# nameofuser1/vad

Hardware: NVIDIA B200
Metric: audio_seconds_per_second (higher is better)
Workload: dtype f32

## Files before the change

### vad_b200/csrc/ffn_tc.cuh

```cuda
#pragma once

#include <cuda_fp16.h>
#include <cuda_runtime.h>

#include <algorithm>
#include <cmath>
#include <cstdint>
#include <cstring>
#include <vector>

#include "vad_core.cuh"

namespace vadb {

constexpr int kTcK1 = 48, kTcN1 = 64;
__host__ __device__ constexpr int tc_feat_col(int feat) {
  const int g = feat / 13, k = feat % 13, q = k / 2, e = k % 2;
  return q < 4 ? 6 * q + 2 * g + e : 24 + 6 * (q - 4) + 2 * g + e;
}
constexpr int kTcK2 = 64, kTcN2 = 32;
constexpr int kTcK3 = 32, kTcN3 = 16;
constexpr int kTcK4 = 16, kTcN4 = 16;
constexpr int kTcBlk1 = kTcK1 * kTcN1 * 4, kTcBlk2 = kTcK2 * kTcN2 * 4, kTcBlk3 = kTcK3 * kTcN3 * 4,
              kTcBlk4 = kTcK4 * kTcN4 * 4;
// ... 194 lines not shown
      "selp.u32 %0, 1, 0, p;\n\t}"
      : "=r"(ok)
      : "r"(tc_smem_u32(bar)), "r"(parity)
      : "memory");
  return ok != 0;
}
__device__ __forceinline__ void tc_mbar_wait(uint64_t* bar, uint32_t parity) {
  while (!tc_mbar_try_wait(bar, parity)) {
  }
}

__device__ __forceinline__ uint64_t tc_smem_desc(uint32_t smem_addr, uint32_t lbo_bytes, uint32_t sbo_bytes) {
  uint64_t d = 0;
  d |= static_cast<uint64_t>((smem_addr >> 4) & 0x3FFF);
  d |= static_cast<uint64_t>((lbo_bytes >> 4) & 0x3FFF) << 16;
  d |= static_cast<uint64_t>((sbo_bytes >> 4) & 0x3FFF) << 32;
  d |= 1ull << 46;
  return d;
}
__host__ __device__ constexpr uint32_t tc_idesc(int n) {
  return (1u << 4)  | (2u << 7)  | (2u << 10)  |
         (static_cast<uint32_t>(n >> 3) << 17) | (static_cast<uint32_t>(128 >> 4) << 24);
}

template <int K, int N>
__device__ __forceinline__ void tc_issue_layer(uint32_t tm_base, uint32_t d_col, uint32_t w_smem, uint64_t* done_bar) {
  constexpr uint32_t lbo = (2 * N / 8) * 128, sbo = 128;
  constexpr uint32_t idesc_2n = tc_idesc(2 * N), idesc_n = tc_idesc(N);
  const uint32_t a_hi = tm_base + kTmA, a_lo = tm_base + kTmA + K, d = tm_base + d_col;
#pragma unroll
  for (int j = 0; j < K / 8; ++j) {
    const uint64_t b = tc_smem_desc(w_smem + 2 * j * lbo, lbo, sbo);
    umma_tf32_ts(d, a_hi + 8 * j, b, idesc_2n, j > 0 ? 1u : 0u);
    umma_tf32_ts(d, a_lo + 8 * j, b, idesc_n, 1u);
  }
  umma_commit(done_bar);
}

__device__ __forceinline__ void tc_split(float x, uint32_t& hi, uint32_t& lo) {
  hi = __float_as_uint(x) & 0xFFFFE000u;
  lo = __float_as_uint(x - __uint_as_float(hi));
}

template <int NOUT, int HALVES>
__device__ __forceinline__ void tc_hidden_epilogue(uint32_t tl, uint32_t d_col, const float* bias, int hidx) {
  constexpr int W = NOUT / HALVES;
  constexpr int CH = W >= 16 ? 16 : 8;
  const int base = hidx * W;
#pragma unroll
  for (int c0 = 0; c0 < W; c0 += CH) {
    uint32_t v[CH], u[CH], hi[CH], lo[CH];
    if constexpr (CH == 16) {
      tmem_ld16(tl + d_col + base + c0, v);
      tmem_ld16(tl + d_col + NOUT + base + c0, u);
    } else {
      tmem_ld8(tl + d_col + base + c0, v);
      tmem_ld8(tl + d_col + NOUT + base + c0, u);
    }
    tmem_wait_ld();
#pragma unroll
    for (int i = 0; i < CH; ++i) {
      const float a = fmaxf((__uint_as_float(v[i]) + __uint_as_float(u[i])) + bias[base + c0 + i], 0.0f);
      tc_split(a, hi[i], lo[i]);
    }
    if constexpr (CH == 16) {
      tmem_st16(tl + kTmA + base + c0, hi);
      tmem_st16(tl + kTmA + NOUT + base + c0, lo);
    } else {
      tmem_st8(tl + kTmA + base + c0, hi);
      tmem_st8(tl + kTmA + NOUT + base + c0, lo);
    }
  }
  tmem_wait_st();
}

template <int HALVES>
__device__ __forceinline__ void tc_bar() {
  if constexpr (HALVES == 2) asm volatile("bar.sync 1, 256;" ::: "memory");
  else asm volatile("bar.sync 1, 128;" ::: "memory");
}

__device__ __forceinline__ void tc_store_a1_half(uint32_t tl, int hidx, const float (&xl)[24]) {
  uint32_t hi[16], lo[16], hi8[8], lo8[8];
#pragma unroll
  for (int i = 0; i < 16; ++i) tc_split(xl[i], hi[i], lo[i]);
#pragma unroll
  for (int i = 0; i < 8; ++i) tc_split(xl[16 + i], hi8[i], lo8[i]);
  const uint32_t b = tl + kTmA + 24 * hidx;
  tmem_st16(b, hi);
  tmem_st8(b + 16, hi8);
  tmem_st16(b + kTcK1, lo);
  tmem_st8(b + kTcK1 + 16, lo8);
}

template <int HALVES>
__device__ __forceinline__ uint32_t ffn_tc_tile(const FfnBias& fb, float (&logit)[kNCls], uint32_t tm_base, int wq, int hidx,
                                                bool is_issuer, uint32_t w_smem, uint64_t* mma_bar, uint32_t par,
                                                long long* ts = nullptr, int dbg = 0) {
  const uint32_t tl = tm_base + (static_cast<uint32_t>(32 * wq) << 16);
#define VADB_TS(i) do { if (ts) ts[i] = clock64(); } while (0)
  tmem_wait_st();
  tc_fence_before();
  tc_bar<HALVES>();
  VADB_TS(3);
  if (is_issuer && !(dbg & 32)) {
    tc_fence_after();
    tc_issue_layer<kTcK1, kTcN1>(tm_base, kTmD1, w_smem + kTcOff1, mma_bar);
  }
  VADB_TS(4);
  if (!(dbg & 32)) { tc_mbar_wait(mma_bar, par); par ^= 1u; }
  tc_fence_after();
  VADB_TS(5);
  if (!(dbg & 128)) tc_hidden_epilogue<kTcN1, HALVES>(tl, kTmD1, fb.b1, hidx);
  VADB_TS(6);
  tc_fence_before();
  tc_bar<HALVES>();
  if (is_issuer && !(dbg & 32)) {
    tc_fence_after();
    tc_issue_layer<kTcK2, kTcN2>(tm_base, kTmD2, w_smem + kTcOff2, mma_bar);
  }
  VADB_TS(7);
  if (!(dbg & 32)) { tc_mbar_wait(mma_bar, par); par ^= 1u; }
  tc_fence_after();
  VADB_TS(8);
  if (!(dbg & 128)) tc_hidden_epilogue<kTcN2, HALVES>(tl, kTmD2, fb.b2, hidx);
  VADB_TS(9);
  tc_fence_before();
  tc_bar<HALVES>();
  if (is_issuer && !(dbg & 32)) {
    tc_fence_after();
    tc_issue_layer<kTcK3, kTcN3>(tm_base, kTmD3, w_smem + kTcOff3, mma_bar);
  }
  VADB_TS(10);
  if (!(dbg & 32)) { tc_mbar_wait(mma_bar, par); par ^= 1u; }
  tc_fence_after();
  VADB_TS(11);
  if (!(dbg & 128)) tc_hidden_epilogue<kTcN3, HALVES>(tl, kTmD3, fb.b3, hidx);
  VADB_TS(12);
  tc_fence_before();
  tc_bar<HALVES>();
  if (is_issuer && !(dbg & 32)) {
    tc_fence_after();
    tc_issue_layer<kTcK4, kTcN4>(tm_base, kTmD4, w_smem + kTcOff4, mma_bar);
  }
  VADB_TS(13);
  if (!(dbg & 32)) { tc_mbar_wait(mma_bar, par); par ^= 1u; }
  tc_fence_after();
  VADB_TS(14);
  if (hidx == 0) {
    uint32_t v[8], u[8];
    tmem_ld8(tl + kTmD4, v);
    tmem_ld8(tl + kTmD4 + kTcN4, u);
    tmem_wait_ld();
#pragma unroll
    for (int o = 0; o < kNCls; ++o) logit[o] = (__uint_as_float(v[o]) + __uint_as_float(u[o])) + fb.b4[o];
  }
  tc_fence_before();
  VADB_TS(15);
#undef VADB_TS
  return par;
}

__device__ __forceinline__ void umma_f16_ts(uint32_t d_tmem, uint32_t a_tmem, uint64_t b_desc, uint32_t idesc,
                                            uint32_t accumulate) {
  asm volatile(
      "{\n\t.reg .pred p;\n\t"
      "setp.ne.b32 p, %4, 0;\n\t"
      "tcgen05.mma.cta_group::1.kind::f16 [%0], [%1], %2, %3, p;\n\t}" ::"r"(d_tmem),
      "r"(a_tmem), "l"(b_desc), "r"(idesc), "r"(accumulate)
      : "memory");
}
__host__ __device__ constexpr uint32_t tc16_idesc(int n) {
  return (1u << 4)  | (static_cast<uint32_t>(n >> 3) << 17) |
         (static_cast<uint32_t>(128 >> 4) << 24);
}
template <int K, int N>
__device__ __forceinline__ void tc16_issue_layer(uint32_t tm_base, uint32_t d_col, uint32_t w_smem, uint64_t* done_bar) {
  constexpr uint32_t lbo = (2 * N / 8) * 128, sbo = 128;
  constexpr uint32_t idesc_2n = tc16_idesc(2 * N), idesc_n = tc16_idesc(N);
  const uint32_t a_hi = tm_base + kTmA, a_lo = tm_base + kTmA + K / 2, d = tm_base + d_col;
#pragma unroll
  for (int j = 0; j < K / 16; ++j) {
    const uint64_t b = tc_smem_desc(w_smem + 2 * j * lbo, lbo, sbo);
    umma_f16_ts(d, a_hi + 8 * j, b, idesc_2n, j > 0 ? 1u : 0u);
    umma_f16_ts(d, a_lo + 8 * j, b, idesc_n, 1u);
  }
  umma_commit(done_bar);
}
__device__ __forceinline__ void tc16_split2(f2 x, uint32_t& hi, uint32_t& lo) {
  const __half2 h = __floats2half2_rn(x.x, x.y);
  const float2 hf = __half22float2(h);
  const f2 r = vsub(x, mk2(hf.x, hf.y));
  const __half2 l = __floats2half2_rn(r.x, r.y);
  hi = *reinterpret_cast<const uint32_t*>(&h);
  lo = *reinterpret_cast<const uint32_t*>(&l);
}
template <int NOUT, int HALVES>
__device__ __forceinline__ void tc16_hidden_epilogue(uint32_t tl, uint32_t d_col, const float* cbias, float postp,
                                                     int hidx) {
  constexpr int W = NOUT / HALVES;
  constexpr int CH = W >= 16 ? 16 : 8;
  const int base = hidx * W;
#pragma unroll
  for (int c0 = 0; c0 < W; c0 += CH) {
    uint32_t v[CH], u[CH], hi[CH / 2], lo[CH / 2];
    if constexpr (CH == 16) {
      tmem_ld16(tl + d_col + base + c0, v);
      tmem_ld16(tl + d_col + NOUT + base + c0, u);
    } else {
      tmem_ld8(tl + d_col + base + c0, v);
      tmem_ld8(tl + d_col + NOUT + base + c0, u);
    }
    tmem_wait_ld();
#pragma unroll
    for (int i = 0; i < CH; i += 2) {
      const f2 d = vadd(mk2(__uint_as_float(v[i]), __uint_as_float(v[i + 1])),
                        mk2(__uint_as_float(u[i]), __uint_as_float(u[i + 1])));
      f2 a = vfma(d, mk2(postp, postp), mk2(cbias[base + c0 + i], cbias[base + c0 + i + 1]));
      a.x = fmaxf(a.x, 0.0f);
      a.y = fmaxf(a.y, 0.0f);
      tc16_split2(a, hi[i / 2], lo[i / 2]);
    }
    if constexpr (CH == 16) {
      tmem_st8(tl + kTmA + (base + c0) / 2, hi);
      tmem_st8(tl + kTmA + NOUT / 2 + (base + c0) / 2, lo);
    } else {
      tmem_st4(tl + kTmA + (base + c0) / 2, hi);
      tmem_st4(tl + kTmA + NOUT / 2 + (base + c0) / 2, lo);
    }
  }
  tmem_wait_st();
}
__device__ __forceinline__ void tc16_store_a1_half(uint32_t tl, int hidx, const float (&xl)[24]) {
  uint32_t hi[8], lo[8], hi4[4], lo4[4];
#pragma unroll
  for (int i = 0; i < 8; ++i) tc16_split2(mk2(xl[2 * i], xl[2 * i + 1]), hi[i], lo[i]);
#pragma unroll
  for (int i = 0; i < 4; ++i) tc16_split2(mk2(xl[16 + 2 * i], xl[17 + 2 * i]), hi4[i], lo4[i]);
  const uint32_t b = tl + kTmA + 12 * hidx;
  tmem_st8(b, hi);
  tmem_st4(b + 8, hi4);
  tmem_st8(b + kTcK1 / 2, lo);
  tmem_st4(b + kTcK1 / 2 + 8, lo4);
}
template <int HALVES>
__device__ __forceinline__ uint32_t ffn_tc16_tile(const FfnBias& fb, float (&logit)[kNCls], uint32_t tm_base, int wq,
                                                  int hidx, bool is_issuer, uint32_t w_smem, uint64_t* mma_bar,
                                                  uint32_t par) {
  const uint32_t tl = tm_base + (static_cast<uint32_t>(32 * wq) << 16);
  tmem_wait_st();
  tc_fence_before();
  tc_bar<HALVES>();
  if (is_issuer) {
    tc_fence_after();
    tc16_issue_layer<kTcK1, kTcN1>(tm_base, kTmD1, w_smem + kTc16Off1, mma_bar);
  }
  tc_mbar_wait(mma_bar, par); par ^= 1u;
  tc_fence_after();
  tc16_hidden_epilogue<kTcN1, HALVES>(tl, kTmD1, fb.c1, fb.postp[0], hidx);
  tc_fence_before();
  tc_bar<HALVES>();
  if (is_issuer) {
    tc_fence_after();
    tc16_issue_layer<kTcK2, kTcN2>(tm_base, kTmD2, w_smem + kTc16Off2, mma_bar);
  }
  tc_mbar_wait(mma_bar, par); par ^= 1u;
  tc_fence_after();
  tc16_hidden_epilogue<kTcN2, HALVES>(tl, kTmD2, fb.c2, fb.postp[1], hidx);
  tc_fence_before();
  tc_bar<HALVES>();
  if (is_issuer) {
    tc_fence_after();
    tc16_issue_layer<kTcK3, kTcN3>(tm_base, kTmD3, w_smem + kTc16Off3, mma_bar);
  }
  tc_mbar_wait(mma_bar, par); par ^= 1u;
  tc_fence_after();
  tc16_hidden_epilogue<kTcN3, HALVES>(tl, kTmD3, fb.c3, fb.postp[2], hidx);
  tc_fence_before();
  tc_bar<HALVES>();
  if (is_issuer) {
    tc_fence_after();
    tc16_issue_layer<kTcK4, kTcN4>(tm_base, kTmD4, w_smem + kTc16Off4, mma_bar);
  }
  tc_mbar_wait(mma_bar, par); par ^= 1u;
  tc_fence_after();
  if (hidx == 0) {
    uint32_t v[8], u[8];
    tmem_ld8(tl + kTmD4, v);
    tmem_ld8(tl + kTmD4 + kTcN4, u);
    tmem_wait_ld();
#pragma unroll
    for (int o = 0; o < kNCls; ++o) logit[o] = fmaf(__uint_as_float(v[o]) + __uint_as_float(u[o]), fb.post[3], fb.b4[o]);
  }
  tc_fence_before();
  return par;
}

constexpr int kTm2Tile = 128;
constexpr int kTm2D1 = 64, kTm2D2 = 64, kTm2D3 = 64, kTm2D4 = 96;
static_assert(2 * kTm2Tile == kTmemCols && kTm2D1 + kTcN1 <= kTm2Tile && kTm2D2 + 2 * kTcN2 <= kTm2Tile &&
              kTm2D4 + 2 * kTcN4 <= kTm2Tile && kTcK2 <= kTm2D1, "two tiles share the CTA's TMEM allocation");

template <int K, int N, bool ONE_ACC>
__device__ __forceinline__ void tc16_issue_layer2(uint32_t tm_base, uint32_t d_col, uint32_t w_smem, bool two_tiles,
                                                  uint64_t* done_bar) {
  constexpr uint32_t lbo = (2 * N / 8) * 128, sbo = 128, lo_off = (N / 8) * 128;
  constexpr int kMmas = ONE_ACC ? 3 : 2;
#pragma unroll
  for (int j = 0; j < K / 16; ++j) {
    const uint32_t b = w_smem + 2 * j * lbo;
    const uint64_t b_hi = tc_smem_desc(b, lbo, sbo), b_lo = tc_smem_desc(b + lo_off, lbo, sbo);
#pragma unroll
    for (int m = 0; m < kMmas; ++m) {
      const uint32_t a_col = kTmA + (m == kMmas - 1 ? K / 2 : 0) + 8 * j;
      const uint64_t bd = (ONE_ACC && m == 1) ? b_lo : b_hi;
      const uint32_t idesc = (!ONE_ACC && m == 0) ? tc16_idesc(2 * N) : tc16_idesc(N);
      const uint32_t acc = (j > 0 || m > 0) ? 1u : 0u;
      umma_f16_ts(tm_base + d_col, tm_base + a_col, bd, idesc, acc);
      if (two_tiles) umma_f16_ts(tm_base + kTm2Tile + d_col, tm_base + kTm2Tile + a_col, bd, idesc, acc);
    }
  }
  umma_commit(done_bar);
}
template <int NOUT>
__device__ __forceinline__ void tc16_epilogue_1acc(uint32_t tl, uint32_t d_col, const float* cbias, float postp) {
#pragma unroll
  for (int c0 = 0; c0 < NOUT; c0 += 16) {
    uint32_t v[16], hi[8], lo[8];
    tmem_ld16(tl + d_col + c0, v);
    tmem_wait_ld();
#pragma unroll
    for (int i = 0; i < 16; i += 2) {
      f2 a = vfma(mk2(__uint_as_float(v[i]), __uint_as_float(v[i + 1])), mk2(postp, postp),
                  mk2(cbias[c0 + i], cbias[c0 + i + 1]));
      a.x = fmaxf(a.x, 0.0f);
      a.y = fmaxf(a.y, 0.0f);
      tc16_split2(a, hi[i / 2], lo[i / 2]);
    }
    tmem_st8(tl + kTmA + c0 / 2, hi);
    tmem_st8(tl + kTmA + NOUT / 2 + c0 / 2, lo);
  }
  tmem_wait_st();
}
__device__ __forceinline__ uint32_t ffn_tc16_tile2_lane(uint32_t tm_base, int warp) {
  return tm_base + kTm2Tile * static_cast<uint32_t>(warp >> 2) + (static_cast<uint32_t>(32 * (warp & 3)) << 16);
}
__device__ __forceinline__ uint32_t ffn_tc16_tile2(const FfnBias& fb, float (&logit)[kNCls], uint32_t tm_base, int warp,
                                                   bool two_tiles, bool is_issuer, uint32_t w_smem, uint64_t* mma_bar,
                                                   uint32_t par, long long* ts = nullptr) {
  const uint32_t tl = ffn_tc16_tile2_lane(tm_base, warp);
#define VADB_TS(i) do { if (ts) ts[i] = clock64(); } while (0)
  tmem_wait_st();
  tc_fence_before();
  tc_bar<2>();
  VADB_TS(3);
  if (is_issuer) {
    tc_fence_after();
    tc16_issue_layer2<kTcK1, kTcN1, true>(tm_base, kTm2D1, w_smem + kTc16Off1, two_tiles, mma_bar);
  }
  VADB_TS(4);
  tc_mbar_wait(mma_bar, par); par ^= 1u;
  tc_fence_after();
  VADB_TS(5);
  tc16_epilogue_1acc<kTcN1>(tl, kTm2D1, fb.c1, fb.postp[0]);
  VADB_TS(6);
  tc_fence_before();
  tc_bar<2>();
  if (is_issuer) {
    tc_fence_after();
    tc16_issue_layer2<kTcK2, kTcN2, false>(tm_base, kTm2D2, w_smem + kTc16Off2, two_tiles, mma_bar);
  }
  VADB_TS(7);
  tc_mbar_wait(mma_bar, par); par ^= 1u;
  tc_fence_after();
  VADB_TS(8);
  tc16_hidden_epilogue<kTcN2, 1>(tl, kTm2D2, fb.c2, fb.postp[1], 0);
  VADB_TS(9);
  tc_fence_before();
  tc_bar<2>();
  if (is_issuer) {
    tc_fence_after();
    tc16_issue_layer2<kTcK3, kTcN3, false>(tm_base, kTm2D3, w_smem + kTc16Off3, two_tiles, mma_bar);
  }
  VADB_TS(10);
  tc_mbar_wait(mma_bar, par); par ^= 1u;
  tc_fence_after();
  VADB_TS(11);
  tc16_hidden_epilogue<kTcN3, 1>(tl, kTm2D3, fb.c3, fb.postp[2], 0);
  VADB_TS(12);
  tc_fence_before();
  tc_bar<2>();
  if (is_issuer) {
    tc_fence_after();
    tc16_issue_layer2<kTcK4, kTcN4, false>(tm_base, kTm2D4, w_smem + kTc16Off4, two_tiles, mma_bar);
  }
  VADB_TS(13);
  tc_mbar_wait(mma_bar, par); par ^= 1u;
  tc_fence_after();
  VADB_TS(14);
  {
    uint32_t v[8], u[8];
    tmem_ld8(tl + kTm2D4, v);
    tmem_ld8(tl + kTm2D4 + kTcN4, u);
    tmem_wait_ld();
#pragma unroll
    for (int o = 0; o < kNCls; ++o) logit[o] = fmaf(__uint_as_float(v[o]) + __uint_as_float(u[o]), fb.post[3], fb.b4[o]);
  }
  tc_fence_before();
  VADB_TS(15);
#undef VADB_TS
  return par;
}
#endif

}
```

### vad_b200/csrc/vad_kernels.cuh

```cuda
#pragma once

#include <cuda_runtime.h>

#include "vad_core.cuh"
#include "ffn_tc.cuh"

namespace vadb {

constexpr int kThreads = 256;
constexpr int kWarps = 8;
constexpr int kStepFrames = 32;
constexpr int kRing = 288;
constexpr int kPPitch = 34;
constexpr int kStageSamples = (kStepFrames - 1) * kHop + kFrame;
constexpr int kStagePad = 5376;
constexpr int kBlockSteps = 8;

constexpr int kOffPcm = 0;
constexpr int kOffExch = kOffPcm + 2 * kStagePad * 2;
constexpr int kOffP = kOffExch + kWarps * 2 * kExchFrame * 8;
constexpr int kP2Bytes = (kP2RowsAlloc * kP2Pitch * 4 + 15) & ~15;
constexpr int kOffLogE = kOffP + kP2Bytes;
constexpr int kLogEFloats = kNMel * 32;
constexpr int kOffRing = kOffLogE + 2 * kLogEFloats * 4;
constexpr int kOffTw1 = kOffRing + ((kRingRows * ring_pitch(kRing) * 4 + 15) & ~15);
constexpr int kOffTw2 = kOffTw1 + 256 * 8;
constexpr int kOffBar = kOffTw2 + 128 * 8;
constexpr int kOffSeg = kOffBar + 48;
constexpr int kFusedSmemBytes = kOffSeg + 16;
constexpr int kBlockStepsTc = 4;
static_assert(kBlockSteps * kStepFrames + 4 <= kRing, "the MFCC ring must hold a whole block phase's windows");
static_assert(kTcBlobBytes <= kWarps * 2 * kExchFrame * 8 + kP2Bytes, "weight blob must fit exch + P");
static_assert(kBlockSteps * kStepFrames * kNFeat * 4 + 16 <= kWarps * 2 * kExchFrame * 8 + kP2Bytes,
              "dataset-row staging tile must fit exch + P");
static_assert(2 * (kFusedSmemBytes + 1024) <= 233472, "two CTAs per SM");

struct Segment {
  long long pcm_start;
  long long out_start;
  int n_frames;
  int cont;
};

struct FrontEnd {
  const cf2* win;
  float preemph;
};

#if defined(VADB_DEBUG_HOOKS)
#define VADB_DBG(p) ((p).debug_skip)
#else
#define VADB_DBG(p) 0
#endif

struct FusedParams {
  const int16_t* pcm;
  long long pcm_len;
  const Segment* segs;
  int seg_begin, seg_end;
  int* counter;
  const cf2* tw1;
  const cf2* tw2;
  uint8_t* labels;
  float* logits;
  float* feats;
  float* rows;
  long long row_base;
  int feat_mode;
  const unsigned char* tc_blob;
  long long* dbg_ts;
  int debug_skip;
};

__device__ __forceinline__ uint32_t smem_u32(const void* p) {
  return static_cast<uint32_t>(__cvta_generic_to_shared(p));
}
__device__ __forceinline__ void mbar_init(uint64_t* bar, uint32_t count) {
  asm volatile("mbarrier.init.shared::cta.b64 [%0], %1;" ::"r"(smem_u32(bar)), "r"(count) : "memory");
}
__device__ __forceinline__ void fence_mbar_init() {
  asm volatile("fence.mbarrier_init.release.cluster;" ::: "memory");
}
__device__ __forceinline__ void mbar_arrive_expect_tx(uint64_t* bar, uint32_t bytes) {
  asm volatile("mbarrier.arrive.expect_tx.shared::cta.b64 _, [%0], %1;" ::"r"(smem_u32(bar)), "r"(bytes)
               : "memory");
}
__device__ __forceinline__ void mbar_arrive(uint64_t* bar) {
  asm volatile("mbarrier.arrive.shared::cta.b64 _, [%0];" ::"r"(smem_u32(bar)) : "memory");
}
__device__ __forceinline__ void warp_arrive(uint64_t* bar, int lane) {
  __syncwarp();
  if (lane == 0) mbar_arrive(bar);
}
__device__ __forceinline__ bool mbar_try_wait(uint64_t* bar, uint32_t parity) {
  uint32_t ok;
  asm volatile(
      "{\n\t.reg .pred p;\n\t"
      "mbarrier.try_wait.parity.shared::cta.b64 p, [%1], %2;\n\t"
      "selp.u32 %0, 1, 0, p;\n\t}"
      : "=r"(ok)
      : "r"(smem_u32(bar)), "r"(parity)
      : "memory");
  return ok != 0;
}
__device__ __forceinline__ void mbar_wait(uint64_t* bar, uint32_t parity) {
  while (!mbar_try_wait(bar, parity)) {
  }
}
__device__ __forceinline__ void bulk_g2s(void* dst_smem, const void* src_gmem, uint32_t bytes, uint64_t* bar) {
  asm volatile(
      "cp.async.bulk.shared::cluster.global.mbarrier::complete_tx::bytes [%0], [%1], %2, [%3];" ::"r"(
          smem_u32(dst_smem)),
      "l"(src_gmem), "r"(bytes), "r"(smem_u32(bar))
      : "memory");
}

struct ShflXchg {
  int lane;
  __device__ __forceinline__ float operator()(float mine, int, bool, int partner) const {
    return __shfl_sync(0xffffffffu, mine, (lane & 16) | partner);
  }
  __device__ __forceinline__ f2 operator()(f2 mine, int, bool, int partner) const {
    const int src = (lane & 16) | partner;
    return mk2(__shfl_sync(0xffffffffu, mine.x, src), __shfl_sync(0xffffffffu, mine.y, src));
  }
};

template <int NZ, class LOAD, class PRE, class STORE>
__device__ __forceinline__ void warp_fft_quad(LOAD&& load, f2* ex, const cf2* s_tw1, const cf2* s_tw2, int lane,
                                               PRE&& before_store, STORE&& store) {
  const int t = lane & 15;
  f2 xr[16], xi[16];
  load(t, xr, xi);
  fft_pass1<NZ>(xr, xi, s_tw1, t);
  exch_store_plane(ex, t, xr);
  __syncwarp();
  exch_load_plane(ex, t, xr);
  __syncwarp();
  exch_store_plane(ex, t, xi);
  __syncwarp();
  exch_load_plane(ex, t, xi);
  __syncwarp();
  dft16<16>(xr, xi);
  before_store();
  fft_split_store(xr, xi, t, s_tw2, ShflXchg{lane}, store);
}
struct P2Store {
  static constexpr bool kHasSink = true;
  float* lo_base;
  float* hi_base;
  float* lo0;
  float* mid_ptr;
  __device__ __forceinline__ P2Store(float* P2, int col, int k1) {
    lo_base = P2 + p2_index(k1, col);
    hi_base = P2 + p2_index(256 - k1, col);
    float* sink = P2 + kP2Rows * kP2Pitch + k1 + 2 * (col & 8);
    lo0 = k1 >= kMelFirstBin ? lo_base : sink;
    mid_ptr = k1 == 0 ? P2 + p2_index(128, col) : sink;
  }
  static __device__ __forceinline__ void put(float* q, f2 v) {
    q[0] = v.x;
    q[2] = v.y;
  }
  template <class K> __device__ __forceinline__ void lo(K, f2 v) const {
    constexpr int k2 = K::value;
    if constexpr (k2 == 0) put(lo0, v);
    else put(lo_base + 8 * k2 * kP2Pitch, v);
  }
  template <class K> __device__ __forceinline__ void hi(K, f2 v) const { put(hi_base - 8 * K::value * kP2Pitch, v); }
  __device__ __forceinline__ void mid(f2 v) const { put(mid_ptr, v); }
};

template <int NZ, class LOAD>
__device__ __forceinline__ void warp_fft_pair(LOAD&& load, cf2* ex, const cf2* s_tw1, const cf2* s_tw2,
                                               float* s_P, int fi, int lane) {
  const int t = lane & 15;
  float xr[16], xi[16];
  load(xr, xi);
  fft_pass1<NZ>(xr, xi, s_tw1, t);
  exch_store(ex, t, xr, xi);
  __syncwarp();
  exch_load(ex, t, xr, xi);
  __syncwarp();
  dft16<16>(xr, xi);
  fft_split_store(xr, xi, t, s_tw2, ShflXchg{lane}, [&](int bin, float v) { s_P[bin * kPPitch + fi] = v; });
}

template <int NTHREADS = kThreads, class GEN>
__device__ __forceinline__ void flush_flat(float* dst, int total, int tid, GEN&& gen) {
  if (total <= 0) return;
  const int head = min(total, static_cast<int>((16u - (reinterpret_cast<uintptr_t>(dst) & 15u)) & 15u) >> 2);
  const int nq = (total - head) >> 2;
  for (int q = tid; q < nq; q += NTHREADS) {
    float v[4];
    gen(head + 4 * q, v, 4);
    *reinterpret_cast<float4*>(dst + head + 4 * q) = make_float4(v[0], v[1], v[2], v[3]);
  }
  const int tail0 = head + 4 * nq;
  if (tid < 2) {
    const int j0 = tid == 0 ? 0 : tail0, cnt = tid == 0 ? head : total - tail0;
    if (cnt > 0) {
      float v[4];
      gen(j0, v, cnt);
#pragma unroll
      for (int i = 0; i < 4; ++i)
        if (i < cnt) dst[j0 + i] = v[i];
    }
  }
}

__device__ __forceinline__ void classify_row(const FfnParams& w, const float (&r)[5][kNCep], int feat_mode,
                                             uint8_t* labels, float* logits, float* feats, long long row, float th) {
  float x[kNFeat];
  const bool ok = window_features(r, feat_mode, x);
  float logit[kNCls];
  ffn_forward(w, x, logit);
  uint8_t lab = decide(logit, th);
  if (!ok) {
    logit[0] = logit[1] = logit[2] = NAN;
    lab = 0;
  }
  if (labels) labels[row] = lab;
  if (logits) {
    logits[row * 3 + 0] = logit[0];
    logits[row * 3 + 1] = logit[1];
    logits[row * 3 + 2] = logit[2];
  }
  if (feats) {
#pragma unroll
    for (int i = 0; i < kNFeat; ++i) feats[row * kNFeat + i] = x[i];
  }
}

template <int MODE, int TC> struct FfnArgOf { using type = FfnNone; };
template <> struct FfnArgOf<2, 0> { using type = FfnParams; };
template <> struct FfnArgOf<2, 1> { using type = FfnBias; };
template <> struct FfnArgOf<2, 2> { using type = FfnBias; };

template <bool FE, class A>
__device__ __forceinline__ uint8_t decide_of(const float (&logit)[kNCls], const A& ffn) {
  if constexpr (FE && !std::is_same<A, FfnNone>::value) return decide(logit, ffn.thresh);
  else return decide(logit);
}

constexpr int kStageOffFe = 8;
static_assert(kStageSamples + kStageOffFe <= kStagePad, "front-end stage offset must fit the PCM buffer");

template <int MODE, int TC, bool FE>
__device__ __forceinline__ void fused_body(const FusedParams& p, const typename FfnArgOf<MODE, TC>::type& ffn,
                                           const FrontEnd& fe, const int tid) {
  static_assert(TC == 0 || MODE == 2, "tensor-core FFN only exists in VAD mode");
  constexpr int kBlk = TC == 1 ? kBlockStepsTc : kBlockSteps;
  constexpr int kStageOff = FE ? kStageOffFe : 0;
  extern __shared__ __align__(128) unsigned char smem[];
  int16_t* s_pcm = reinterpret_cast<int16_t*>(smem + kOffPcm);
  cf2* s_exch = reinterpret_cast<cf2*>(smem + kOffExch);
  float* s_P = reinterpret_cast<float*>(smem + kOffP);
  float* s_logE = reinterpret_cast<float*>(smem + kOffLogE);
  float* s_ring = reinterpret_cast<float*>(smem + kOffRing);
  cf2* s_tw1 = reinterpret_cast<cf2*>(smem + kOffTw1);
  cf2* s_tw2 = reinterpret_cast<cf2*>(smem + kOffTw2);
  uint64_t* s_bar = reinterpret_cast<uint64_t*>(smem + kOffBar);
  int* s_seg = reinterpret_cast<int*>(smem + kOffSeg);

  const int warp = tid >> 5, lane = tid & 31, h = lane >> 4, t = lane & 15;

  s_tw1[tid] = p.tw1[tid];
  if (tid < 128) s_tw2[tid] = p.tw2[tid];
  uint32_t* s_tmem = reinterpret_cast<uint32_t*>(smem + kOffSeg + 8);
  if (tid == 0) {
    mbar_init(&s_bar[0], 1);
    mbar_init(&s_bar[1], 1);
    mbar_init(&s_bar[2], 1);
    mbar_init(&s_bar[3], 1);
    mbar_init(&s_bar[4], kWarps);
    mbar_init(&s_bar[5], kWarps);
    fence_mbar_init();
  }
  uint32_t tm_base = 0, w_par = 0, mma_par = 0;
  int dbg_n = 0;
  if (TC) {
    if (warp == 0) tmem_alloc(s_tmem, kTmemCols);
    tc_fence_before();
    __syncthreads();
    tc_fence_after();
    tm_base = *s_tmem;
  }

  unsigned gstep = 0;
  Segment seg{};
  const P2Store p2store(s_P, col_of_halfwarp(warp, h), t);
  __syncthreads();
  warp_arrive(&s_bar[4], lane);


  auto issue_load = [&](int step, int buf) {
    const long long start = seg.pcm_start + static_cast<long long>(step) * (kStepFrames * kHop);
    const long long avail = p.pcm_len - start;
    const int nsmp = avail >= kStageSamples ? kStageSamples : (avail > 0 ? static_cast<int>(avail) : 0);
    const int bulk = (nsmp * 2) & ~15;
    int16_t* dst = s_pcm + buf * kStagePad + kStageOff;
    if (tid == 0) {
      mbar_arrive_expect_tx(&s_bar[buf], static_cast<uint32_t>(bulk));
      if (bulk) bulk_g2s(dst, p.pcm + start, static_cast<uint32_t>(bulk), &s_bar[buf]);
    }
    const int tail0 = bulk >> 1;
    if (tid < nsmp - tail0) dst[tail0 + tid] = p.pcm[start + tail0 + tid];
    if (FE && tid == 31) dst[-1] = (step > 0 || seg.cont) ? p.pcm[start - 1] : int16_t(0);
  };

  for (;;) {
    __syncthreads();
    if (tid == 0) *s_seg = p.seg_begin + atomicAdd(p.counter, 1);
    __syncthreads();
    const int si = *s_seg;
    if (si >= p.seg_end) break;
    seg = p.segs[si];
    const int n = seg.n_frames;
    const int nsteps = (n + kStepFrames - 1) / kStepFrames;
    int out_done = (MODE == 0) ? 0 : 2;
    bool dct_pending = false;
    if (nsteps > 0 && warp == 0) issue_load(0, gstep & 1);
    __syncthreads();

    for (int s = 0; s < nsteps; ++s, ++gstep) {
      const int buf = gstep & 1;
      if (s + 1 < nsteps && warp == 0) issue_load(s + 1, buf ^ 1);
      mbar_wait(&s_bar[buf], (gstep >> 1) & 1);

      const uint32_t par = gstep & 1;
      auto dct_step = [&](int sd) {
        if (!(VADB_DBG(p) & 4)) {
          const float* le = s_logE + (sd & 1) * kLogEFloats + lane;
          const int col = (sd * kStepFrames + slot_of_col(lane)) % kRing;
          if (warp < 3) {
            float ra, rb, rc, rd;
            dct_coef4<32>(le, 2 * warp, ra, rb, rc, rd);
            *reinterpret_cast<float2*>(s_ring + ring_idx(4 * warp, col, kRing)) = make_float2(ra, rb);
            *reinterpret_cast<float2*>(s_ring + ring_idx(4 * warp + 2, col, kRing)) = make_float2(rc, rd);
          } else if (warp == 3) {
            float ra, rb;
            dct_coef2<32>(le, 6, ra, rb);
            s_ring[ring_idx(12, col, kRing)] = ra;
          }
        }
      };

      const uint32_t* stage32 = reinterpret_cast<const uint32_t*>(s_pcm + buf * kStagePad + kStageOff);
      if (!(VADB_DBG(p) & 1)) {
        f2* ex = reinterpret_cast<f2*>(s_exch) + (warp * 2 + h) * kExchFrame;
        const uint32_t* w32a = stage32 + (warp * 4 + h) * (kHop / 2);
        warp_fft_quad<13>(
            [&](int tt, f2 (&xr)[16], f2 (&xi)[16]) {
              if constexpr (FE) fft_load_pcm2_fe(w32a, kHop, tt, fe.preemph, fe.win, xr, xi);
              else fft_load_pcm2(w32a, kHop, tt, xr, xi);
            },
            ex, s_tw1, s_tw2, lane, [&] { mbar_wait(&s_bar[4], par); }, p2store);
      } else {
        mbar_wait(&s_bar[4], par);
      }
      warp_arrive(&s_bar[5], lane);

      if (dct_pending) dct_step(s - 1);
      mbar_wait(&s_bar[5], par);

      if (!(VADB_DBG(p) & 2))
        mel2_run_dispatch<kP2Pitch, 32>(warp, s_P + 2 * lane, s_logE + (s & 1) * kLogEFloats + lane);
      warp_arrive(&s_bar[4], lane);
      const int computed = min((s + 1) * kStepFrames, n);
      const bool block_now = (((s + 1) % kBlk) == 0 || s == nsteps - 1) && !(VADB_DBG(p) & 8);
      const bool tc_now = TC && block_now && (computed - 2 - out_done) > 0;
      dct_pending = !block_now;

      if (block_now) {
        if (tc_now) asm volatile("fence.proxy.async.shared::cta;" ::: "memory");
        __syncthreads();
        if (tc_now && tid == 0 && !(VADB_DBG(p) & 16)) {
          constexpr uint32_t blob_bytes = TC == 2 ? kTc16BlobBytes : kTcBlobBytes;
          mbar_arrive_expect_tx(&s_bar[2], blob_bytes);
          bulk_g2s(smem + kOffExch, p.tc_blob, blob_bytes, &s_bar[2]);
        }
        dct_step(s);
      }

      if (block_now) {
        __syncthreads();
        if (MODE == 0) {
          float* dst = p.rows + (seg.out_start - p.row_base + out_done) * kNCep;
          const int first = out_done;
          flush_flat(dst, (computed - out_done) * kNCep, tid, [&](int j, float (&v)[4], int cnt) {
            int fr = j / kNCep, cf = j - fr * kNCep;
#pragma unroll
            for (int i = 0; i < 4; ++i) {
              if (i < cnt) v[i] = s_ring[ring_idx(cf, (first + fr) % kRing, kRing)];
              if (++cf == kNCep) { cf = 0; ++fr; }
            }
          });
          out_done = computed;
        } else if (MODE == 1) {
          const int n_valid = computed - 2 - out_done;
          if (n_valid > 0) {
            float* dst = p.rows + (seg.out_start - p.row_base + (out_done - 2)) * kNFeat;
            float* stage = reinterpret_cast<float*>(smem + kOffExch) + ((reinterpret_cast<uintptr_t>(dst) & 15u) >> 2);
            if (tid < n_valid) {
              float xa[24], xb[24];
              window_features_pairs<0, 4, kRing, 24>(s_ring, out_done + tid, 1, xa);
              window_features_pairs<4, 7, kRing, 24>(s_ring, out_done + tid, 1, xb);
              float* row = stage + tid * kNFeat;
#pragma unroll
              for (int g = 0; g < 3; ++g) {
#pragma unroll
                for (int k = 0; k < 8; ++k) row[g * kNCep + k] = xa[6 * (k >> 1) + 2 * g + (k & 1)];
#pragma unroll
                for (int k = 0; k < 5; ++k) row[g * kNCep + 8 + k] = xb[6 * (k >> 1) + 2 * g + (k & 1)];
              }
            }
            __syncthreads();
            flush_flat(dst, n_valid * kNFeat, tid, [&](int j, float (&v)[4], int cnt) {
              if (cnt == 4) {
                const float4 q = *reinterpret_cast<const float4*>(stage + j);
                v[0] = q.x; v[1] = q.y; v[2] = q.z; v[3] = q.w;
              } else {
#pragma unroll
                for (int i = 0; i < 4; ++i)
                  if (i < cnt) v[i] = stage[j + i];
              }
            });
            __syncthreads();
          }
          out_done = max(out_done, computed - 2);
        } else if (!TC) {
          const int c = out_done + tid;
          if (c <= computed - 3) {
            float r[5][kNCep];
#pragma unroll
            for (int d = 0; d < 5; ++d) {
              const int col = (c - 2 + d) % kRing;
#pragma unroll
              for (int k = 0; k < kNCep; ++k) r[d][k] = s_ring[ring_idx(k, col, kRing)];
            }
            if constexpr (MODE == 2 && TC == 0)
              classify_row(ffn, r, p.feat_mode, p.labels, p.logits, p.feats, seg.out_start - p.row_base + (c - 2),
                           FE ? ffn.thresh : 0.0f);
          }
          out_done = max(out_done, computed - 2);
        } else if constexpr (TC == 2) {
          const int n_valid = computed - 2 - out_done;
          if (n_valid > 0) {
            long long* ts = nullptr;
#if defined(VADB_DEBUG_HOOKS)
            if (p.dbg_ts && blockIdx.x == 0 && tid == 0 && dbg_n < 64) ts = p.dbg_ts + 16 * dbg_n;
#endif
            if (ts) ts[0] = clock64();
            const bool valid = tid < n_valid;
            const int c = out_done + (valid ? tid : 0);
            const long long row = seg.out_start - p.row_base + (c - 2);
            const uint32_t tl = ffn_tc16_tile2_lane(tm_base, warp);
            bool ok = true;
#pragma unroll
            for (int hidx = 0; hidx < 2; ++hidx) {
              float xl[24];
              if (VADB_DBG(p) & 64) {
#pragma unroll
                for (int i = 0; i < 24; ++i) xl[i] = 0.5f;
              } else {
                ok = (hidx == 0 ? window_features_pairs<0, 4, kRing, 24>(s_ring, c, p.feat_mode, xl)
                                : window_features_pairs<4, 7, kRing, 24>(s_ring, c, p.feat_mode, xl)) && ok;
              }
              tc16_store_a1_half(tl, hidx, xl);
              if (p.feats && valid) {
                const int k0 = hidx ? 8 : 0, nk = hidx ? 5 : 8;
#pragma unroll
                for (int k = 0; k < 8; ++k)
#pragma unroll
                  for (int g = 0; g < 3; ++g)
                    if (k < nk) p.feats[row * kNFeat + g * kNCep + k0 + k] = xl[6 * (k >> 1) + 2 * g + (k & 1)];
              }
            }
            if (ts) ts[1] = clock64();
            if (!(VADB_DBG(p) & 16)) mbar_wait(&s_bar[2], w_par);
            if (ts) ts[2] = clock64();
            float logit[kNCls];
            const bool two_tiles = n_valid > 128 && !(VADB_DBG(p) & 256);
            mma_par = ffn_tc16_tile2(ffn, logit, tm_base, warp, two_tiles, tid == 0, smem_u32(smem + kOffExch), &s_bar[3],
                                     mma_par, ts);
            ++dbg_n;
            if (valid) {
              uint8_t lab = decide_of<FE>(logit, ffn);
              if (!ok) {
                logit[0] = logit[1] = logit[2] = NAN;
                lab = 0;
              }
              p.labels[row] = lab;
              if (p.logits) {
                p.logits[row * 3 + 0] = logit[0];
                p.logits[row * 3 + 1] = logit[1];
                p.logits[row * 3 + 2] = logit[2];
              }
            }
            if (!(VADB_DBG(p) & 16)) w_par ^= 1u;
            __syncthreads();
          }
          out_done = max(out_done, computed - 2);
        } else {
          const int n_valid = computed - 2 - out_done;
          if (n_valid > 0) {
            unsigned char* wdst = smem + kOffExch;
            {
              const int fr = tid & 127, hidx = tid >> 7;
              long long* ts = nullptr;
#if defined(VADB_DEBUG_HOOKS)
              if (p.dbg_ts && blockIdx.x == 0 && tid == 0 && dbg_n < 64) ts = p.dbg_ts + 16 * dbg_n;
#endif
              if (ts) ts[0] = clock64();
              const bool valid = fr < n_valid;
              const int c = out_done + (valid ? fr : 0);
              const uint32_t tl = tm_base + (static_cast<uint32_t>(32 * (warp & 3)) << 16);
              float xl[24], logit[kNCls];
              bool ok_half = true;
              if (VADB_DBG(p) & 64) {
#pragma unroll
                for (int i = 0; i < 24; ++i) xl[i] = 0.5f;
              } else {
                ok_half = (hidx == 0) ? window_features_pairs<0, 4, kRing, 24>(s_ring, c, p.feat_mode, xl)
                                      : window_features_pairs<4, 7, kRing, 24>(s_ring, c, p.feat_mode, xl);
              }
              s_logE[tid] = ok_half ? 1.0f : 0.0f;
              if (ts) ts[1] = clock64();
              tc_store_a1_half(tl, hidx, xl);
              if (p.feats && valid) {
                const long long row = seg.out_start - p.row_base + (c - 2);
                const int k0 = hidx ? 8 : 0, nk = hidx ? 5 : 8;
#pragma unroll
                for (int k = 0; k < 8; ++k)
#pragma unroll
                  for (int g = 0; g < 3; ++g)
                    if (k < nk) p.feats[row * kNFeat + g * kNCep + k0 + k] = xl[6 * (k >> 1) + 2 * g + (k & 1)];
              }
              if (!(VADB_DBG(p) & 16)) mbar_wait(&s_bar[2], w_par);
              if (ts) ts[2] = clock64();
              if constexpr (TC == 1)
                mma_par = ffn_tc_tile<2>(ffn, logit, tm_base, warp & 3, hidx, tid == 0, smem_u32(wdst), &s_bar[3], mma_par,
                                         ts, VADB_DBG(p));
              ++dbg_n;
              if (valid && hidx == 0) {
                const bool ok = s_logE[fr] != 0.0f && s_logE[128 + fr] != 0.0f;
                uint8_t lab = decide_of<FE>(logit, ffn);
                if (!ok) {
                  logit[0] = logit[1] = logit[2] = NAN;
                  lab = 0;
                }
                const long long row = seg.out_start - p.row_base + (c - 2);
                p.labels[row] = lab;
                if (p.logits) {
                  p.logits[row * 3 + 0] = logit[0];
                  p.logits[row * 3 + 1] = logit[1];
                  p.logits[row * 3 + 2] = logit[2];
                }
              }
            }
            if (!(VADB_DBG(p) & 16)) w_par ^= 1u;
            __syncthreads();
          }
          out_done = max(out_done, computed - 2);
        }
      }
    }
  }
  if (TC) {
    tc_fence_before();
    __syncthreads();
    if (warp == 0) tmem_dealloc(tm_base, kTmemCols);
  }
  if (tid == 0) {
    __threadfence();
    if (atomicAdd(p.counter + 1, 1) == static_cast<int>(gridDim.x) - 1) {
      p.counter[0] = 0;
      p.counter[1] = 0;
      __threadfence();
    }
  }
}

template <int MODE, int TC>
__global__ void __launch_bounds__(kThreads, 2) fused_kernel(const __grid_constant__ FusedParams p,
                                                            const __grid_constant__ typename FfnArgOf<MODE, TC>::type ffn) {
  fused_body<MODE, TC, false>(p, ffn, FrontEnd{nullptr, 0.0f}, threadIdx.x);
}
template <int MODE, int TC>
__global__ void __launch_bounds__(kThreads, 2) fused_fe_kernel(const __grid_constant__ FusedParams p,
                                                               const __grid_constant__ typename FfnArgOf<MODE, TC>::type ffn,
                                                               const __grid_constant__ FrontEnd fe) {
  fused_body<MODE, TC, true>(p, ffn, fe, threadIdx.x);
}

constexpr int kFfnTcSmemBytes = kTcBlobBytes + 64;
template <int KIND>
__global__ void __launch_bounds__(128) ffn_tc_rows_kernel(const float* x, long long n, const unsigned char* blob16,
                                                          const unsigned char* blob32, uint8_t* labels, float* logits,
                                                          const __grid_constant__ FfnBias fb) {
  extern __shared__ __align__(128) unsigned char smem[];
  uint64_t* bars = reinterpret_cast<uint64_t*>(smem + kTcBlobBytes);
  uint32_t* s_tmem = reinterpret_cast<uint32_t*>(smem + kTcBlobBytes + 32);
  const int tid = threadIdx.x, warp = tid >> 5;
  if (tid == 0) {
    mbar_init(&bars[0], 1);
    mbar_init(&bars[1], 1);
    fence_mbar_init();
  }
  if (warp == 0) tmem_alloc(s_tmem, kTmemCols);
  tc_fence_before();
  __syncthreads();
  tc_fence_after();
  const uint32_t tm_base = *s_tmem;
  if (KIND == 1 && tid == 0) {
    mbar_arrive_expect_tx(&bars[0], kTcBlobBytes);
    bulk_g2s(smem, blob32, kTcBlobBytes, &bars[0]);
  }
  const long long i = static_cast<long long>(blockIdx.x) * 128 + tid;
  const long long src = i < n ? i : n - 1;
  float v[kNFeat], logit[kNCls];
  bool ok = true, wide = false;
#pragma unroll
  for (int k = 0; k < kNFeat; ++k) {
    v[k] = x[src * kNFeat + k];
    ok = ok && (fabsf(v[k]) <= 3.0e38f);
    if constexpr (KIND == 2)
      wide = wide || fabsf(v[k]) > (k < kNCep ? kFeatBoundZ : k < 2 * kNCep ? kFeatBoundD1 : kFeatBoundD2);
  }
  bool fp16 = false;
  if constexpr (KIND == 2) {
    fp16 = !__syncthreads_or(wide);
    if (tid == 0) {
      const uint32_t bytes = fp16 ? kTc16BlobBytes : kTcBlobBytes;
      mbar_arrive_expect_tx(&bars[0], bytes);
      bulk_g2s(smem, fp16 ? blob16 : blob32, bytes, &bars[0]);
    }
  }
  mbar_wait(&bars[0], 0);
  {
    const uint32_t tl = tm_base + (static_cast<uint32_t>(32 * warp) << 16);
    float h0[24], h1[24];
#pragma unroll
    for (int i = 0; i < 24; ++i) h0[i] = h1[i] = 0.0f;
#pragma unroll
    for (int f = 0; f < kNFeat; ++f) {
      const int col = tc_feat_col(f);
      if (col < 24) h0[col] = v[f];
      else h1[col - 24] = v[f];
    }
    if (fp16) {
      tc16_store_a1_half(tl, 0, h0);
      tc16_store_a1_half(tl, 1, h1);
    } else {
      tc_store_a1_half(tl, 0, h0);
      tc_store_a1_half(tl, 1, h1);
    }
  }
  if (fp16) ffn_tc16_tile<1>(fb, logit, tm_base, warp, 0, tid == 0, smem_u32(smem), &bars[1], 0);
  else ffn_tc_tile<1>(fb, logit, tm_base, warp, 0, tid == 0, smem_u32(smem), &bars[1], 0);
  if (i < n) {
    uint8_t lab = decide(logit, fb.thresh);
    if (!ok) {
      logit[0] = logit[1] = logit[2] = NAN;
      lab = 0;
    }
    if (labels) labels[i] = lab;
    if (logits) {
      logits[i * 3 + 0] = logit[0];
      logits[i * 3 + 1] = logit[1];
      logits[i * 3 + 2] = logit[2];
    }
  }
  tc_fence_before();
  __syncthreads();
  if (warp == 0) tmem_dealloc(tm_base, kTmemCols);
}

#if defined(VADB_DEBUG_HOOKS)
constexpr int kExpSmemBytes = 2 * kStagePad * 2 + kWarps * 2 * kExchFrame * 8 + 384 * 8 + 64;
template <int MINB>
__global__ void __launch_bounds__(kThreads, MINB) exp_fft_kernel(const FusedParams p, float* sink) {
  extern __shared__ __align__(128) unsigned char smem[];
  int16_t* s_pcm = reinterpret_cast<int16_t*>(smem);
  cf2* s_exch = reinterpret_cast<cf2*>(smem + 2 * kStagePad * 2);
  cf2* s_tw1 = reinterpret_cast<cf2*>(smem + 2 * kStagePad * 2 + kWarps * 2 * kExchFrame * 8);
  cf2* s_tw2 = s_tw1 + 256;
  uint64_t* s_bar = reinterpret_cast<uint64_t*>(s_tw2 + 128);
  int* s_seg = reinterpret_cast<int*>(s_bar + 4);
  const int tid = threadIdx.x, warp = tid >> 5, lane = tid & 31, h = lane >> 4, t = lane & 15;
  s_tw1[tid] = p.tw1[tid];
  if (tid < 128) s_tw2[tid] = p.tw2[tid];
  if (tid == 0) {
    mbar_init(&s_bar[0], 1);
    mbar_init(&s_bar[1], 1);
    fence_mbar_init();
  }
  unsigned gstep = 0;
  float acc = 0.0f;
  Segment seg;
  auto issue_load = [&](int step, int buf) {
    const long long start = seg.pcm_start + static_cast<long long>(step) * (kStepFrames * kHop);
    const long long avail = p.pcm_len - start;
    const int nsmp = avail >= kStageSamples ? kStageSamples : (avail > 0 ? static_cast<int>(avail) : 0);
    const int bulk = (nsmp * 2) & ~15;
    if (tid == 0) {
      mbar_arrive_expect_tx(&s_bar[buf], static_cast<uint32_t>(bulk));
      if (bulk) bulk_g2s(s_pcm + buf * kStagePad, p.pcm + start, static_cast<uint32_t>(bulk), &s_bar[buf]);
    }
  };
  for (;;) {
    __syncthreads();
    if (tid == 0) *s_seg = p.seg_begin + atomicAdd(p.counter, 1);
    __syncthreads();
    const int si = *s_seg;
    if (si >= p.seg_end) break;
    seg = p.segs[si];
    const int nsteps = (seg.n_frames + kStepFrames - 1) / kStepFrames;
    issue_load(0, gstep & 1);
    __syncthreads();
    for (int s = 0; s < nsteps; ++s, ++gstep) {
      const int buf = gstep & 1;
      if (s + 1 < nsteps) issue_load(s + 1, buf ^ 1);
      mbar_wait(&s_bar[buf], (gstep >> 1) & 1);
      const uint32_t* stage32 = reinterpret_cast<const uint32_t*>(s_pcm + buf * kStagePad);
      cf2* ex = s_exch + (warp * 2 + h) * kExchFrame;
#pragma unroll 1
      for (int r = 0; r < 2; ++r) {
        const int fi = warp * 4 + r * 2 + h;
        const uint32_t* w32 = stage32 + fi * (kHop / 2);
        float xr[16], xi[16];
        fft_load_pcm(w32, t, xr, xi);
        fft_pass1<13>(xr, xi, s_tw1, t);
        exch_store(ex, t, xr, xi);
        __syncwarp();
        exch_load(ex, t, xr, xi);
        __syncwarp();
        dft16<16>(xr, xi);
        fft_split_store(xr, xi, t, s_tw2, ShflXchg{lane}, [&](int bin, float v) { acc = fmaf(v, 1e-12f * bin, acc); });
      }
      __syncthreads();
    }
  }
  if (acc == 123.456f) sink[0] = acc;
}
#endif

constexpr int kFramesSmemBytes = kWarps * 2 * kExchFrame * 8 + kBins * kPPitch * 4 + kNMel * 32 * 4 + 384 * 8;

__global__ void __launch_bounds__(kThreads) frames_kernel(const float* frames, long long n, int frame_len, int what,
                                                         float* out, const cf2* tw1, const cf2* tw2, FrontEnd fe) {
  extern __shared__ __align__(128) unsigned char smem[];
  cf2* s_exch = reinterpret_cast<cf2*>(smem);
  float* s_P = reinterpret_cast<float*>(smem + kWarps * 2 * kExchFrame * 8);
  float* s_logE = s_P + kBins * kPPitch;
  cf2* s_tw1 = reinterpret_cast<cf2*>(s_logE + kNMel * 32);
  cf2* s_tw2 = s_tw1 + 256;
  const int tid = threadIdx.x, warp = tid >> 5, lane = tid & 31, h = lane >> 4, t = lane & 15;
  s_tw1[tid] = tw1[tid];
  if (tid < 128) s_tw2[tid] = tw2[tid];
  __syncthreads();
  const long long f0 = static_cast<long long>(blockIdx.x) * kStepFrames;
  cf2* ex = s_exch + (warp * 2 + h) * kExchFrame;
#pragma unroll 1
  for (int r = 0; r < 2; ++r) {
    const int fi = warp * 4 + r * 2 + h;
    const long long f = min(f0 + fi, n - 1);
    const float* fr = frames + f * frame_len;
    warp_fft_pair<16>(
        [&](float (&xr)[16], float (&xi)[16]) {
          if (fe.win) fft_load_f32_fe(fr, frame_len, t, fe.preemph, fe.win, xr, xi);
          else fft_load_f32(fr, frame_len, t, xr, xi);
        },
        ex, s_tw1, s_tw2, s_P, fi, lane);
  }
  __syncthreads();
  if (what == 0) {
    for (int j = tid; j < kStepFrames * kBins; j += kThreads) {
      const int fi = j >> 8, k = j & 255;
      if (f0 + fi < n) out[(f0 + fi) * kBins + k] = s_P[k * kPPitch + fi] * 9.5367431640625e-07f;
    }
    return;
  }
  mel_group_dispatch<kPPitch, 32>(warp, s_P + lane, s_logE + lane);
  __syncthreads();
  if (f0 + lane < n) {
    out[(f0 + lane) * kNCep + warp] = dct_coef<32>(s_logE + lane, warp);
// ... 434 lines not shown
```

Baseline: 21.22 million.

## Decouple the two FFN tensor-core tiles with per-tile barriers and issuers

The two 128-row tiles of the tensor-core FFN used to be driven by one issuing thread and a CTA-wide barrier per layer. Now each group of four warps runs its own tile: its own named barrier (bar.sync 1 or 2 with 128 threads), its own MMA-completion mbarrier (a new s_bar[6]) and its own issuer thread. The aim is to let one tile's epilogue overlap the other tile's MMAs and to avoid whole-CTA syncs; when only one tile is valid, the second group's warps skip the FFN entirely. The risk is that per-thread parity tracking becomes per-tile and now depends on those skipped iterations staying consistent.

```diff
diff --git a/vad_b200/csrc/ffn_tc.cuh b/vad_b200/csrc/ffn_tc.cuh
--- a/vad_b200/csrc/ffn_tc.cuh
+++ b/vad_b200/csrc/ffn_tc.cuh
@@ -520,8 +520,7 @@
               kTm2D4 + 2 * kTcN4 <= kTm2Tile && kTcK2 <= kTm2D1, "two tiles share the CTA's TMEM allocation");
 
 template <int K, int N, bool ONE_ACC>
-__device__ __forceinline__ void tc16_issue_layer2(uint32_t tm_base, uint32_t d_col, uint32_t w_smem, bool two_tiles,
-                                                  uint64_t* done_bar) {
+__device__ __forceinline__ void tc16_issue_layer2(uint32_t tm_base, uint32_t d_col, uint32_t w_smem, uint64_t* done_bar) {
   constexpr uint32_t lbo = (2 * N / 8) * 128, sbo = 128, lo_off = (N / 8) * 128;
   constexpr int kMmas = ONE_ACC ? 3 : 2;
 #pragma unroll
@@ -535,7 +534,6 @@
       const uint32_t idesc = (!ONE_ACC && m == 0) ? tc16_idesc(2 * N) : tc16_idesc(N);
       const uint32_t acc = (j > 0 || m > 0) ? 1u : 0u;
       umma_f16_ts(tm_base + d_col, tm_base + a_col, bd, idesc, acc);
-      if (two_tiles) umma_f16_ts(tm_base + kTm2Tile + d_col, tm_base + kTm2Tile + a_col, bd, idesc, acc);
     }
   }
   umma_commit(done_bar);
@@ -563,57 +561,70 @@
 __device__ __forceinline__ uint32_t ffn_tc16_tile2_lane(uint32_t tm_base, int warp) {
   return tm_base + kTm2Tile * static_cast<uint32_t>(warp >> 2) + (static_cast<uint32_t>(32 * (warp & 3)) << 16);
 }
+__device__ __forceinline__ void tc16_tile_bar(int tile) {
+  if (tile == 0) asm volatile("bar.sync 1, 128;" ::: "memory");
+  else asm volatile("bar.sync 2, 128;" ::: "memory");
+}
 __device__ __forceinline__ uint32_t ffn_tc16_tile2(const FfnBias& fb, float (&logit)[kNCls], uint32_t tm_base, int warp,
-                                                   bool two_tiles, bool is_issuer, uint32_t w_smem, uint64_t* mma_bar,
-                                                   uint32_t par, long long* ts = nullptr) {
+                                                   bool two_tiles, uint32_t w_smem, uint64_t* mma_bar0,
+                                                   uint64_t* mma_bar1, uint32_t par, long long* ts = nullptr) {
+  const int tile = warp >> 2;
+  if (tile == 1 && !two_tiles) {
+#pragma unroll
+    for (int o = 0; o < kNCls; ++o) logit[o] = 0.0f;
+    return par;
+  }
+  const bool is_issuer = (warp & 3) == 0 && (threadIdx.x & 31) == 0;
   const uint32_t tl = ffn_tc16_tile2_lane(tm_base, warp);
+  const uint32_t tb = tm_base + kTm2Tile * static_cast<uint32_t>(tile);
+  uint64_t* bar = tile ? mma_bar1 : mma_bar0;
 #define VADB_TS(i) do { if (ts) ts[i] = clock64(); } while (0)
   tmem_wait_st();
   tc_fence_before();
-  tc_bar<2>();
+  tc16_tile_bar(tile);
   VADB_TS(3);
   if (is_issuer) {
     tc_fence_after();
-    tc16_issue_layer2<kTcK1, kTcN1, true>(tm_base, kTm2D1, w_smem + kTc16Off1, two_tiles, mma_bar);
+    tc16_issue_layer2<kTcK1, kTcN1, true>(tb, kTm2D1, w_smem + kTc16Off1, bar);
   }
   VADB_TS(4);
-  tc_mbar_wait(mma_bar, par); par ^= 1u;
+  tc_mbar_wait(bar, par); par ^= 1u;
   tc_fence_after();
   VADB_TS(5);
   tc16_epilogue_1acc<kTcN1>(tl, kTm2D1, fb.c1, fb.postp[0]);
   VADB_TS(6);
   tc_fence_before();
-  tc_bar<2>();
-  if (is_issuer) {
-    tc_fence_after();
-    tc16_issue_layer2<kTcK2, kTcN2, false>(tm_base, kTm2D2, w_smem + kTc16Off2, two_tiles, mma_bar);
+  tc16_tile_bar(tile);
+  if (is_issuer) {
+    tc_fence_after();
+    tc16_issue_layer2<kTcK2, kTcN2, false>(tb, kTm2D2, w_smem + kTc16Off2, bar);
   }
   VADB_TS(7);
-  tc_mbar_wait(mma_bar, par); par ^= 1u;
+  tc_mbar_wait(bar, par); par ^= 1u;
   tc_fence_after();
   VADB_TS(8);
   tc16_hidden_epilogue<kTcN2, 1>(tl, kTm2D2, fb.c2, fb.postp[1], 0);
   VADB_TS(9);
   tc_fence_before();
-  tc_bar<2>();
-  if (is_issuer) {
-    tc_fence_after();
-    tc16_issue_layer2<kTcK3, kTcN3, false>(tm_base, kTm2D3, w_smem + kTc16Off3, two_tiles, mma_bar);
+  tc16_tile_bar(tile);
+  if (is_issuer) {
+    tc_fence_after();
+    tc16_issue_layer2<kTcK3, kTcN3, false>(tb, kTm2D3, w_smem + kTc16Off3, bar);
   }
   VADB_TS(10);
-  tc_mbar_wait(mma_bar, par); par ^= 1u;
+  tc_mbar_wait(bar, par); par ^= 1u;
   tc_fence_after();
   VADB_TS(11);
   tc16_hidden_epilogue<kTcN3, 1>(tl, kTm2D3, fb.c3, fb.postp[2], 0);
   VADB_TS(12);
   tc_fence_before();
-  tc_bar<2>();
-  if (is_issuer) {
-    tc_fence_after();
-    tc16_issue_layer2<kTcK4, kTcN4, false>(tm_base, kTm2D4, w_smem + kTc16Off4, two_tiles, mma_bar);
+  tc16_tile_bar(tile);
+  if (is_issuer) {
+    tc_fence_after();
+    tc16_issue_layer2<kTcK4, kTcN4, false>(tb, kTm2D4, w_smem + kTc16Off4, bar);
   }
   VADB_TS(13);
-  tc_mbar_wait(mma_bar, par); par ^= 1u;
+  tc_mbar_wait(bar, par); par ^= 1u;
   tc_fence_after();
   VADB_TS(14);
   {
diff --git a/vad_b200/csrc/vad_kernels.cuh b/vad_b200/csrc/vad_kernels.cuh
--- a/vad_b200/csrc/vad_kernels.cuh
+++ b/vad_b200/csrc/vad_kernels.cuh
@@ -26,7 +26,7 @@
 constexpr int kOffTw1 = kOffRing + ((kRingRows * ring_pitch(kRing) * 4 + 15) & ~15);
 constexpr int kOffTw2 = kOffTw1 + 256 * 8;
 constexpr int kOffBar = kOffTw2 + 128 * 8;
-constexpr int kOffSeg = kOffBar + 48;
+constexpr int kOffSeg = kOffBar + 56;
 constexpr int kFusedSmemBytes = kOffSeg + 16;
 constexpr int kBlockStepsTc = 4;
 static_assert(kBlockSteps * kStepFrames + 4 <= kRing, "the MFCC ring must hold a whole block phase's windows");
@@ -275,6 +275,7 @@
     mbar_init(&s_bar[3], 1);
     mbar_init(&s_bar[4], kWarps);
     mbar_init(&s_bar[5], kWarps);
+    mbar_init(&s_bar[6], 1);
     fence_mbar_init();
   }
   uint32_t tm_base = 0, w_par = 0, mma_par = 0;
@@ -482,7 +483,7 @@
             if (ts) ts[2] = clock64();
             float logit[kNCls];
             const bool two_tiles = n_valid > 128 && !(VADB_DBG(p) & 256);
-            mma_par = ffn_tc16_tile2(ffn, logit, tm_base, warp, two_tiles, tid == 0, smem_u32(smem + kOffExch), &s_bar[3],
+            mma_par = ffn_tc16_tile2(ffn, logit, tm_base, warp, two_tiles, smem_u32(smem + kOffExch), &s_bar[3], &s_bar[6],
                                      mma_par, ts);
             ++dbg_n;
             if (valid) {
```

Measured after the change: 21.35 million, median of 6. About the same (+0.6%).
